# steve-the-bayesian/BOOM

Measured on AMD Instinct MI355X. Metric: Gibbs sweeps/sec (all chains), n=1e4 p=512 spike-slab, higher is better.
Workload: dtype f64; 1 GPU; BregVsSampler spike-and-slab n=1e4 p=512, 1024 chains per GPU, fp64 (BASELINE configs[1]); chains_per_gpu=1024, true_signals=16, burn_in=1000, parallelism=chains sharded, 1 GPU(s), suf_build=single device MFMA syrk

## Files before the change

boom_amd/capi.py:

```python
import ctypes as C
import os

import numpy as np

_HERE = os.path.dirname(os.path.abspath(__file__))
LIB_PATH = os.environ.get("BOOM_AMD_LIB", os.path.join(_HERE, "libboomamd.so"))

_dp = C.POINTER(C.c_double)
_u8p = C.POINTER(C.c_uint8)

SUMMARY_SCALARS = 16


class BoomAmdError(RuntimeError):

    def __init__(self, code, message):
        super().__init__(message)
        self.code = code


class BaConfig(C.Structure):
    _fields_ = [("device", C.c_int32), ("chains", C.c_int32),
                ("chain_offset", C.c_int64), ("seed", C.c_uint64),
                ("max_model_size_hint", C.c_int32), ("reserved", C.c_int32)]
# ... 7 lines not shown
    "ba_engine_destroy": (None, [C.c_void_p]),
    "ba_engine_info": (C.c_int, [C.c_void_p, C.POINTER(C.c_int32),
                                 C.POINTER(C.c_int32), C.POINTER(C.c_int32)]),
    "ba_build_suf_from_xy": (C.c_int, [C.c_void_p, C.c_int64, C.c_int32, _dp, _dp]),
    "ba_build_suf_from_xy_device": (C.c_int, [C.c_void_p, C.c_int64, C.c_int32,
                                              C.c_void_p, C.c_void_p]),
    "ba_suf_block_size": (C.c_size_t, [C.c_int32]),
    "ba_suf_partial_device": (C.c_int, [C.c_void_p, C.c_int64, C.c_int32, C.c_void_p,
                                        C.c_void_p, C.c_void_p]),
    "ba_set_suf_from_block_device": (C.c_int, [C.c_void_p, C.c_int64, C.c_int32, C.c_void_p]),
    "ba_upload_regression_suf": (C.c_int, [C.c_void_p, C.c_int32, _dp, _dp,
                                           C.c_double, C.c_double, C.c_double, _dp]),
    "ba_get_regression_suf": (C.c_int, [C.c_void_p, _dp, _dp, _dp, _dp, _dp, _dp]),
    "ba_set_slab": (C.c_int, [C.c_void_p, _dp, _dp]),
    "ba_set_spike": (C.c_int, [C.c_void_p, _dp, C.c_int64]),
    "ba_set_sigma_prior": (C.c_int, [C.c_void_p, C.c_double, C.c_double, C.c_double]),
    "ba_set_priors_ctor1": (C.c_int, [C.c_void_p, C.c_double, C.c_double,
                                      C.c_double, C.c_int32]),
    "ba_set_priors_ctor2": (C.c_int, [C.c_void_p, C.c_double, C.c_double,
                                      C.c_double, C.c_double, C.c_double, C.c_int32]),
    "ba_get_priors": (C.c_int, [C.c_void_p, _dp, _dp, _dp, _dp, _dp]),
    "ba_set_options": (C.c_int, [C.c_void_p, C.c_int32, C.c_double, C.c_int32, C.c_int32]),
    "ba_set_tuning": (C.c_int, [C.c_void_p, C.c_int32, C.c_int32, C.c_int32]),
    "ba_set_lookahead": (C.c_int, [C.c_void_p, C.c_int32]),
    "ba_draw_next": (C.c_int, [C.c_void_p]),
    "ba_set_state": (C.c_int, [C.c_void_p, C.c_int64, _u8p, _dp, C.c_double]),
    "ba_get_state": (C.c_int, [C.c_void_p, C.c_int64, _u8p, _dp, _dp]),
    "ba_get_states": (C.c_int, [C.c_void_p, _u8p, _dp, _dp]),
    "ba_logpri": (C.c_int, [C.c_void_p, C.c_int64, _dp]),
    "ba_seed": (C.c_int, [C.c_void_p, C.c_uint64]),
    "ba_sweep": (C.c_int, [C.c_void_p, C.c_int32]),
    "ba_sync": (C.c_int, [C.c_void_p]),
    "ba_log_model_prob": (C.c_int, [C.c_void_p, C.c_int32, _u8p, _dp]),
    "ba_set_sigsq": (C.c_int, [C.c_void_p, C.c_int64, C.c_double]),
    "ba_sss_set_slab": (C.c_int, [C.c_void_p, _dp, _dp, C.c_int32, C.c_int32]),
    "ba_sss_sweep": (C.c_int, [C.c_void_p, C.c_int32]),
    "ba_adaptive_set_options": (C.c_int, [C.c_void_p, C.c_int32, C.c_double, C.c_double]),
    "ba_adaptive_sweep": (C.c_int, [C.c_void_p, C.c_int32]),
    "ba_adaptive_get_rates": (C.c_int, [C.c_void_p, C.c_int64, _dp, _dp,
                                        C.POINTER(C.c_uint64)]),
    "ba_reset_summaries": (C.c_int, [C.c_void_p]),
    "ba_get_summaries": (C.c_int, [C.c_void_p, _dp, _dp, _dp, _dp]),
    "ba_summaries_device": (C.c_int, [C.c_void_p, C.c_void_p]),
    "ba_enable_traces": (C.c_int, [C.c_void_p, C.c_int32]),
    "ba_get_traces": (C.c_int, [C.c_void_p, C.c_int32, _dp, _dp, _dp]),
    "ba_enable_draws": (C.c_int, [C.c_void_p, C.c_int32]),
# ... 204 lines not shown
    def set_priors_ctor2(self, prior_sigma_nobs, prior_sigma_guess, prior_beta_nobs,
                         diagonal_shrinkage, prior_inclusion_probability,
                         force_intercept=True):
        self._check(self.lib.ba_set_priors_ctor2(
            self._h, prior_sigma_nobs, prior_sigma_guess, prior_beta_nobs,
            diagonal_shrinkage, prior_inclusion_probability, int(force_intercept)))

    def get_priors(self):
        p = self.p
        b, om, pi = np.zeros(p), np.zeros(p * p), np.zeros(p)
        df, ss = C.c_double(), C.c_double()
        self._check(self.lib.ba_get_priors(self._h, _p(b), _p(om), _p(pi),
                                           C.byref(df), C.byref(ss)))
        return dict(b=b, ominv=om.reshape(p, p).T.copy(), pi=pi, df=df.value, ss=ss.value)

    def set_options(self, max_flips=-1, swap_threshold=0.8, draw_beta=True,
                    draw_sigma=True):
        self._check(self.lib.ba_set_options(self._h, max_flips, swap_threshold,
                                            int(draw_beta), int(draw_sigma)))

    def set_tuning(self, waves_per_chain=0, walk_policy=-1, kcap_start=0):
        self._check(self.lib.ba_set_tuning(self._h, waves_per_chain, walk_policy, kcap_start))

    def set_state(self, gamma, beta=None, sigsq=1.0, chain=-1):
        g = np.ascontiguousarray(gamma, dtype=np.uint8)
        bb = None if beta is None else _f64(beta)
        self._check(self.lib.ba_set_state(self._h, chain, _b(g), _p(bb), sigsq))

    def get_state(self, chain):
        p = self.p
        g = np.zeros(p, np.uint8)
        b = np.zeros(p)
        s = C.c_double()
        self._check(self.lib.ba_get_state(self._h, chain, _b(g), _p(b), C.byref(s)))
        return g, b, s.value

    def get_states(self):
        p, c = self.p, self.chains
        g = np.zeros((c, p), np.uint8)
        b = np.zeros((c, p))
        s = np.zeros(c)
        self._check(self.lib.ba_get_states(self._h, _b(g), _p(b), _p(s)))
        return g, b, s

    def seed(self, seed):
        self._check(self.lib.ba_seed(self._h, seed))
# ... 39 lines not shown
    def adaptive_sweep(self, nsweeps=1, sync=True):
        self._check(self.lib.ba_adaptive_sweep(self._h, nsweeps))
        if sync:
            self.sync()

    def adaptive_get_rates(self, chain):
        b, d = np.zeros(self.p), np.zeros(self.p)
        it = C.c_uint64()
        self._check(self.lib.ba_adaptive_get_rates(self._h, chain, _p(b), _p(d), C.byref(it)))
        return b, d, it.value

    def reset_summaries(self):
        self._check(self.lib.ba_reset_summaries(self._h))

    def get_summaries(self):
        p = self.p
        inc, bs, bs2 = np.zeros(p), np.zeros(p), np.zeros(p)
        sc = np.zeros(SUMMARY_SCALARS)
        self._check(self.lib.ba_get_summaries(self._h, _p(inc), _p(bs), _p(bs2), _p(sc)))
        return dict(inclusion_count=inc, beta_sum=bs, beta_sumsq=bs2,
                    sweeps=sc[0], sigsq_sum=sc[1], sigsq_sumsq=sc[2], k_sum=sc[3],
                    accepts=sc[4], proposals=sc[5], min_margin=sc[6],
                    slot_hits=float(sc[7]), phase_cycles=sc[8:16].copy(),
                    min_multi_margin=float(sc[8]))

    def summaries_device(self, ptr):
        self._check(self.lib.ba_summaries_device(self._h, ptr))

    def enable_traces(self, max_sweeps):
        self._check(self.lib.ba_enable_traces(self._h, max_sweeps))

    def logpri(self, chain=0):
        out = C.c_double()
        self._check(self.lib.ba_logpri(self._h, chain, C.byref(out)))
        return out.value

    def enable_draws(self, max_sweeps):
        self._check(self.lib.ba_enable_draws(self._h, max_sweeps))

    def get_draws(self, chain, nsweeps):
        p = self.p
        g = np.zeros((nsweeps, p), np.uint8)
        b = np.zeros((nsweeps, p))
        s = np.zeros(nsweeps)
        self._check(self.lib.ba_get_draws(self._h, chain, nsweeps, _b(g), _p(b), _p(s)))
        return g, b, s

# ... 489 lines not shown
```

boom_amd/csrc/diag.h:

```cpp
#pragma once

#define BA_STAMP_ADD(ph, last, i, now, T) do { const long long t_ = (long long)(now); (ph)[i] += (T)(t_ - (last)); (last) = t_; } while (0)
#define BA_STAMP_OFF do { } while (0)
#define BA_CORE_CLOCK __builtin_readcyclecounter()

struct StampCtx { long long last; double ph[8]; };

#ifdef BA_STAMPS
#define STAMP_DECL long long st_last = (long long)BA_CORE_CLOCK; double st_ph[8] = {0, 0, 0, 0, 0, 0, 0, 0}
#define STAMP(i) BA_STAMP_ADD(st_ph, st_last, i, BA_CORE_CLOCK, double)
#else
#define STAMP_DECL BA_STAMP_OFF
#define STAMP(i) BA_STAMP_OFF
#endif
#if defined(BA_STAMPS) && defined(BA_STAMPS2)
#define SUBSTAMP(c, i) BA_STAMP_ADD((c).ph, (c).last, i, BA_CORE_CLOCK, double)
#else
#define SUBSTAMP(c, i) BA_STAMP_OFF
#endif
#if defined(BA_STAMPS) && defined(BA_STAMPS3)
#define TSTAMP(c, i) BA_STAMP_ADD((c).ph, (c).last, i, BA_CORE_CLOCK, double)
#else
#define TSTAMP(c, i) BA_STAMP_OFF
#endif
#if defined(BA_STAMPS) && defined(BA_STAMPS4)
#define HSTAMP(c, i) BA_STAMP_ADD((c).ph, (c).last, i, BA_CORE_CLOCK, double)
#else
#define HSTAMP(c, i) BA_STAMP_OFF
#endif
#ifdef BA_PSTAMPS
#define PSTAMP(i) pst[i] = (long long)BA_CORE_CLOCK
#else
#define PSTAMP(i) BA_STAMP_OFF
#endif
#ifdef BA_KSTAMPS
#define KSTAMP(i) BA_STAMP_ADD(kph, klast, i, BA_CORE_CLOCK, long long)
#define SSTAMP(i) BA_STAMP_ADD(kph, klast, i, BA_CORE_CLOCK, long long)
#else
#define KSTAMP(i) BA_STAMP_OFF
#define SSTAMP(i) BA_STAMP_OFF
#endif
#ifdef BA_RSTAMPS
#define RSTAMP(i) BA_STAMP_ADD(rph, rlast, i, wall_clock64(), long long)
#else
#define RSTAMP(i) BA_STAMP_OFF
#endif
```

boom_amd/csrc/engine.hip:

```cpp
#include "engine_internal.h"

namespace boom_amd {

static thread_local std::string g_error = "";

int fail(int code, const std::string &msg) {
  g_error = msg;
  return code;
}

}

namespace {


const char *status_message(int st) {
  switch (st) {
    case CHAIN_NOT_PD:
      return "The posterior information matrix is not positive definite.  "
             "Check your data or consider adjusting your prior.";
    case CHAIN_NEGATIVE_SS:
      return "Illegal data caused negative sum of squares in "
             "Breg::set_reg_post_params.";
    case CHAIN_ILLEGAL_START:
// ... 292 lines not shown
  P.todo = e->dtodo.ptr;
  P.maxk = e->dmaxk.ptr;
  P.trace_idx = e->dtrace_idx.ptr;
  P.model_scratch = e->dmodel.ptr;
  P.table_lp = e->dtab_lp.ptr;
  P.table_kind = e->dtab_kind.ptr;
  P.table_tag = e->dtab_tag.ptr;
  P.table_keep = e->table_ok ? 1 : 0;
  P.model_tag = e->dmodel_tag.ptr;
  P.model_keep = e->model_ok ? 1 : 0;
  P.suf_changed = (e->data_kind == DATA_STATE_SPACE || latent_data(e->data_kind)) ? 1 : 0;
  P.run_limit = 0;
  P.ran = nullptr;
  P.model_scratch_stride = (int64_t)ssvs_scalar_layout(64).total;
  P.big_kcap = e->big_kcap;
  P.big_model = e->dbig_model.ptr;
  P.big_model_stride = e->big_kcap > 0 ? (int64_t)ssvs_scalar_layout(e->big_kcap).total : 0;
  P.big_xs = e->dbig_xs.ptr;
  P.seed_lo = (uint32_t)e->seed;
  P.seed_hi = (uint32_t)(e->seed >> 32);
  P.stream = 0;
  P.mode = e->cur_mode;
  P.walk_policy = e->tune_walk_policy >= 0 ? e->tune_walk_policy : 1;
  if (e->cur_mode == 1) {
    P.slab_scales = e->sss_slab_scales;
    P.stream = 3;
    P.rng_pos = e->dpos_sss.ptr;
    P.draw_sigma = 0;
    P.draw_beta = 1;
    P.cm_start = nullptr;
    P.max_flips = (e->sss_max_flips > 0) ? std::min(e->sss_max_flips, e->p) : e->p;
  }
  if (e->cur_mode == 1 && student_kind(e->data_kind) && !e->student_allow_selection)
    P.max_flips = 0;
  if (e->cur_mode == 1 && column_service(e->data_kind) && e->cols.V.count) {
    P.mode = e->data_kind == DATA_LOGIT ? 2 : 1;
    if (e->data_kind == DATA_MLOGIT) {
      P.mode = 3;
      P.flip_order = e->dml_order.ptr;
      P.wss = e->dml_wss.ptr;
      if (!e->mlogit_select) P.max_flips = 0;
    }
    P.V = e->cols.V.ptr;
    P.v_chain_stride = (int64_t)e->p * e->p;
    P.model_keep = 0;
    P.table_keep = 0;
// ... 872 lines not shown
  e->swap_threshold = swap_threshold;
  e->draw_beta = draw_beta;
  e->draw_sigma = draw_sigma;
  return BA_OK;
}

int ba_set_tuning(ba_engine *e, int32_t waves_per_chain, int32_t walk_policy,
                  int32_t kcap_start) {
  if (!e) return fail(BA_E_INVALID, "null engine");
  if (!(waves_per_chain == 0 || waves_per_chain == 1 || waves_per_chain == 2 || waves_per_chain == 4))
    return fail(BA_E_INVALID, "waves_per_chain must be 0, 1, 2 or 4");
  if (walk_policy < -1 || walk_policy > 3) return fail(BA_E_INVALID, "walk_policy must be in [-1, 3]");
  if (kcap_start < 0) return fail(BA_E_INVALID, "kcap_start must be non-negative");
  MUTATE(e);
  if (e->state_ready) {
    int rc = set_device(e);
    if (!rc) rc = ba_sync(e);
    if (rc) return rc;
  }
  e->tune_waves = waves_per_chain;
  e->tune_walk_policy = walk_policy;
  e->tune_kcap_start = kcap_start;
  e->device_dirty = true;
  return BA_OK;
}

int ba_set_slot_limit(ba_engine *e, int32_t uniforms) {
  if (!e) return fail(BA_E_INVALID, "null engine");
  if (uniforms < 0 || (uniforms & 1)) return fail(BA_E_INVALID, "uniforms must be even and non-negative");
  MUTATE(e);
  e->slot_limit = uniforms;
  return BA_OK;
}

int ba_set_state(ba_engine *e, int64_t chain, const uint8_t *gamma,
                 const double *beta, double sigsq) {
  ENGINE_PROLOGUE(e);
  if (e->p <= 0) return fail(BA_E_STATE, "set the regression data first");
  if (!gamma) return fail(BA_E_INVALID, "null argument");
  const int64_t C = e->cfg.chains;
  if (chain < -1 || chain >= C) return fail(BA_E_INVALID, "chain index out of range");
  if (latent_data(e->data_kind) && !student_kind(e->data_kind) && sigsq != 1.0)
    return fail(BA_E_INVALID, "the binomial samplers' latent data have unit variance: sigsq must be 1");
  if (chain < 0) la_discard(e);
  MUTATE(e);
  if (e->state_ready) {
// ... 873 lines not shown
```

boom_amd/csrc/engine_internal.h:

```cpp
#pragma once
#include <hip/hip_runtime.h>

#include <algorithm>
#include <cmath>
#include <cstdio>
#include <cstdlib>
#include <cstring>
#include <limits>
#include <string>
#include <unordered_map>
#include <vector>

#include "../../include/boom_amd.h"
#include "kalman_params.h"
#include "ktimer.h"
#include "mlogit_params.h"
#include "probit_params.h"
#include "products.h"
#include "quantile_params.h"
#include "ssvs_params.h"
#include "student_params.h"

namespace boom_amd {
hipError_t launch_ssvs_sweep(hipStream_t stream, const SsvsParams &P, int nsweeps);
// ... 169 lines not shown
    int len = 1, avail = 0, served = 0;
    struct Rows { std::vector<double> k, sig, beta; std::vector<uint16_t> idx; };
    std::unordered_map<int64_t, Rows> cache;
    bool synced = false;
    bool pipe = true;
    bool cur_piped = false;
    bool ahead = false;
    int slot = 0;
    hipEvent_t done[2] = {nullptr, nullptr};
    struct Snap {
      DevBuf<uint8_t> gamma;
      DevBuf<double> beta, sigsq, bsum, bsumsq, acc;
      DevBuf<uint16_t> perm;
      DevBuf<uint64_t> pos;
      DevBuf<int32_t> fail;
      DevBuf<uint32_t> inc;
    } snap;
  } la;
  int rec_cap = 64;
  bool big_active = false;
  int big_kcap = 0;
  DevBuf<double> dbig_model, dbig_xs;
  int tune_waves = 0, tune_walk_policy = -1, tune_kcap_start = 0;
  int cur_mode = 0;
  int sss_slab_scales = 1;
  int sss_max_flips = -1;
  double v_scale = 1.0;
  double v_scale_want = 1.0;
  DevBuf<uint64_t> dpos_sss;
  uint64_t seed = 0;
  DevBuf<double> dada_birth, dada_death, dada_ws;
  DevBuf<uint64_t> dada_iter, dpos_ada;
  int ada_max_flips = 100;
  double ada_step = .001, ada_target = .345;

  bool ss_level_set = false, ss_initialized = false;
  int T = 0;
  DevBuf<double> dss_y, dss_X, dss_scratch;
  void *pinned = nullptr;
  size_t pinned_bytes = 0;
  uint64_t api_seq = 1, clean_seq = 0;
  int api_depth = 0;
  DevBuf<double> dss_yt, dss_Xt;
  DevBuf<uint32_t> dss_obs_mask;
  DevBuf<uint8_t> dss_obs;
  DevBuf<double> dxty_c, dyty_c, dnobs_c;
// ... 199 lines not shown
```

boom_amd/csrc/ssvs_device.h:

```cpp
#pragma once
#include <hip/hip_runtime.h>

#include "device_rng.h"
#include "diag.h"
#include "ssvs_params.h"

namespace boom_amd {

namespace {

constexpr int WAVE = 64;
#define BA_INF (__builtin_inf())


#define AS_LDS __attribute__((address_space(3)))
typedef AS_LDS double lds_f64;
typedef AS_LDS uint16_t lds_u16;
typedef AS_LDS uint32_t lds_u32;
typedef AS_LDS uint8_t lds_u8;
template <class T>
__device__ __forceinline__ AS_LDS T *to_lds(unsigned char *generic) {
  return (AS_LDS T *)(uintptr_t)generic;
}
#define AS_CONST __attribute__((address_space(4)))
// ... 96 lines not shown
};

__device__ __forceinline__ void bind_lds(Chain &ch, unsigned char *smem,
                                         const SsvsLds &lay) {
  ch.Lv = to_lds<double>(smem + lay.Lv);
  ch.La = to_lds<double>(smem + lay.La);
  ch.rdv = to_lds<double>(smem + lay.rdv);
  ch.rda = to_lds<double>(smem + lay.rda);
  ch.w = to_lds<double>(smem + lay.w);
  ch.bg = to_lds<double>(smem + lay.bg);
  ch.g = to_lds<uint16_t>(smem + lay.g);
  ch.perm = to_lds<uint16_t>(smem + lay.perm0);
  ch.perm_alt = to_lds<uint16_t>(smem + lay.perm1);
  ch.oth = to_lds<uint16_t>(smem + lay.oth);
  ch.last = to_lds<uint32_t>(smem + lay.last);
  ch.pred = to_lds<uint16_t>(smem + lay.pred);
  ch.gam = to_lds<uint8_t>(smem + lay.gam);
  ch.gam0 = to_lds<uint8_t>(smem + lay.gam0);
  ch.nbr = to_lds<uint8_t>(smem + lay.nbr);
}

__device__ __forceinline__ void chol_blocks2(const Chain &ch, lds_f64 *LA, lds_f64 *rdA,
                                             lds_f64 *LV, lds_f64 *rdV, bool *okA,
                                             bool *okV, double *ldA, double *ldV) {
  const int k = ch.k, i = ch.lane;
  bool oa = true, ov = true;
  for (int j = 0; j < k && (oa || ov); ++j) {
    const bool mine = (i >= j) && (i < k);
    const int ii = mine ? i : j;
    const int jb = j >> 3;
    const int offi = ((ii >> 3) * ((ii >> 3) + 1) / 2) * 64 + (ii & 7) * 8;
    const int offj = (jb * (jb + 1) / 2) * 64 + (j & 7) * 8;
    double sa = LA[bidx(ii, j)], sv = LV[bidx(ii, j)];
    for (int nb = 0; nb < jb; ++nb) {
      typedef double d2_t __attribute__((ext_vector_type(2)));
      const AS_LDS d2_t *pa = (const AS_LDS d2_t *)(LA + offi + nb * 64), *pb = (const AS_LDS d2_t *)(LA + offj + nb * 64);
      const AS_LDS d2_t *pc = (const AS_LDS d2_t *)(LV + offi + nb * 64), *pd = (const AS_LDS d2_t *)(LV + offj + nb * 64);
      d2_t a[4], b[4], c[4], d[4];
#pragma unroll
      for (int t = 0; t < 4; ++t) { a[t] = pa[t]; b[t] = pb[t]; c[t] = pc[t]; d[t] = pd[t]; }
#pragma unroll
      for (int t = 0; t < 4; ++t) {
        sa -= a[t].x * b[t].x;
        sv -= c[t].x * d[t].x;
        sa -= a[t].y * b[t].y;
        sv -= c[t].y * d[t].y;
      }
    }
    {
      const int rem = j & 7;
// ... 26 lines not shown
    }
    if (ov) {
      if (i == j) {
        LV[bidx(j, j)] = sdv;
        rdV[j] = 1.0 / sdv;
      } else if (mine) {
        LV[bidx(i, j)] = sv / sdv;
      }
    }
    wave_sync();
  }
  double la = 0.0, lv = 0.0;
  const double lga = (oa && i < k) ? log(LA[bidx(i, i)]) : 0.0;
  const double lgv = (ov && i < k) ? log(LV[bidx(i, i)]) : 0.0;
  for (int j = 0; j < k; ++j) {
    la += bcast_u(lga, j);
    lv += bcast_u(lgv, j);
  }
  *okA = oa; *okV = ov;
  *ldA = 2.0 * la; *ldV = 2.0 * lv;
}

template <bool REUSE, bool MLVS = false>
__device__ __forceinline__ void refactor(const SsvsParams &P, Chain &ch, Model &M, StampCtx &sx) {
  const int lane = ch.lane, p = ch.p, k = ch.k;
  M.bad = 0;
  M.pd = true;
  double lp;
  const double ldv_in = M.ldv, lda_in = M.lda;
  wave_sync();
  const int kpad = (k + 7) & ~7;
  const int nelem = REUSE ? 0 : kpad * (kpad + 1) / 2;
  const int gm = (lane < k) ? ch.g[lane] : 0;
  const double bm = (lane < k) ? P.b[gm] : 0.0;
  const double xg = (lane < k) ? ch.xty[gm] : 0.0;
  int m0 = 0, n0 = 0;
  double v0 = 0.0, a0 = 0.0;
  if (!REUSE && lane < nelem) {
    int m = (int)((sqrtf(8.0f * (float)lane + 1.0f) - 1.0f) * 0.5f);
    while ((m + 1) * (m + 2) / 2 <= lane) ++m;
    while (m * (m + 1) / 2 > lane) --m;
    m0 = m;
    n0 = lane - m * (m + 1) / 2;
    if (m < k) {
      const size_t o = (size_t)ch.g[m] * p + ch.g[n0];
      v0 = P.V[o] * ch.sv;
      a0 = P.A[o] * ch.sa;
    }
  }
  if (REUSE) {
    lp = M.lp;
  } else {
    double t0 = 0.0, t1 = 0.0;
    if (lane < p) t0 = ch.gam[lane] ? P.l1[lane] : P.l0[lane];
    if (lane + WAVE < p) t1 = ch.gam[lane + WAVE] ? P.l1[lane + WAVE] : P.l0[lane + WAVE];
    double part = 0.0;
    if (lane < p) part += t0;
    if (lane + WAVE < p) part += t1;
    for (int j = lane + 2 * WAVE; j < p; j += WAVE) part += ch.gam[j] ? P.l1[j] : P.l0[j];
    lp = wave_sum(part);
    if (P.max_model_size >= 0 && k > P.max_model_size) lp = -BA_INF;
    if (!(lp > -BA_INF)) lp = -BA_INF;
  }
  M.lp = lp;
  M.ldv = M.lda = M.Q = M.c = 0.0;
  M.SS = ch.ss0q;
  if (k == 0) {
    if constexpr (MLVS) M.logp = lp + ch.k0add;
    else M.logp = ch.mode ? lp : lp - (0.5 * ch.DF - 1.0) * log(ch.ss0q);
    return;
  }
  if (lp == -BA_INF) {
    M.logp = -BA_INF;
    M.pd = false;
    return;
  }
  if (!REUSE && lane < nelem) {
    ch.Lv[bidx(m0, n0)] = v0;
    ch.La[bidx(m0, n0)] = a0;
  }
  for (int e = lane + WAVE; e < nelem; e += WAVE) {
    int m = (int)((sqrtf(8.0f * (float)e + 1.0f) - 1.0f) * 0.5f);
    while ((m + 1) * (m + 2) / 2 <= e) ++m;
    while (m * (m + 1) / 2 > e) --m;
    const int n = e - m * (m + 1) / 2;
    double v = 0.0, a = 0.0;
    if (m < k) {
      const size_t o = (size_t)ch.g[m] * p + ch.g[n];
      v = P.V[o] * ch.sv;
      a = P.A[o] * ch.sa;
    }
    ch.Lv[bidx(m, n)] = v;
    ch.La[bidx(m, n)] = a;
  }
  if (!REUSE && lane < kpad) {
    ch.bg[lane] = bm;
    if (lane >= k) {
      ch.rdv[lane] = 0.0;
      ch.rda[lane] = 0.0;
      ch.w[lane] = 0.0;
    }
  }
  double ab = 0.0;
  unsigned long long nz = __ballot(bm != 0.0);
  while (nz) {
    const int n = __ffsll((long long)nz) - 1;
    nz &= nz - 1;
    const double bn = bcast_u(bm, n);
    const int gn = bcast_u(gm, n);
    if (lane < k) ab += (P.A[(size_t)gm * p + gn] * ch.sa) * bn;
  }
  const double r = (lane < k) ? ab + xg * ch.sx : 0.0;
  M.c = wave_sum(lane < k ? bm * ab : 0.0);
  wave_sync();
  bool okv = true, oka = true;
  if (REUSE) {
    M.lda = lda_in;
    M.ldv = ldv_in;
  } else {
    chol_blocks2(ch, ch.La, ch.rda, ch.Lv, ch.rdv, &oka, &okv, &M.lda, &M.ldv);
  }
  if (!okv) {
    M.pd = false;
    M.logp = -BA_INF;
    return;
  }
  double x = r;
  const double rdm = (lane < k) ? ch.rdv[lane] : 0.0;
#pragma nounroll
  for (int jb = 0; jb * 8 < k; ++jb) {
    double lr[8];
    const int rowm = (lane >= jb * 8 && lane < k) ? lane : jb * 8;
    const int base = bidx(rowm, jb * 8);
#pragma unroll
    for (int t = 0; t < 8; ++t) lr[t] = ch.Lv[base + t];
#pragma unroll
    for (int t = 0; t < 8; ++t) {
      const int j = jb * 8 + t;
      if (j < k) {
        const double wj = bcast_u(x, j) * bcast_u(rdm, j);
        if (lane == j) x = wj;
        else if (lane > j && lane < k) x -= lr[t] * wj;
      }
    }
// ... 4 lines not shown
  wave_sync();
  if (ch.mode) {
    if (!oka) {
      M.lda = -BA_INF;
      M.logp = -BA_INF;
      return;
    }
    M.logp = lp + 0.5 * (M.lda - M.ldv) - 0.5 * (M.c - M.Q);
    return;
  }
  if (!(M.SS >= 0.0) || isinf(M.SS)) {
    M.bad = CHAIN_NEGATIVE_SS;
    M.logp = -BA_INF;
    return;
  }
  if (!oka) {
    M.lda = -BA_INF;
    M.logp = -BA_INF;
    return;
  }
  M.logp = lp + 0.5 * (M.lda - M.ldv) - (0.5 * ch.DF - 1.0) * log(M.SS);
}

__device__ __forceinline__ void apply_flip(Chain &ch, int j) {
  const int lane = ch.lane, k = ch.k;
  const int gm = (lane < k) ? ch.g[lane] : 0x7fffffff;
  const int below = __popcll(__ballot(lane < k && gm < j));
  const bool add = !ch.gam[j];
  wave_sync();
  if (add) {
    const int up = __shfl_up(gm, 1, WAVE);
    if (lane == below) ch.g[lane] = (uint16_t)j;
    else if (lane > below && lane <= k) ch.g[lane] = (uint16_t)up;
    if (lane == 0) ch.gam[j] = 1;
    ch.k = k + 1;
  } else {
    const int dn = __shfl_down(gm, 1, WAVE);
    if (lane >= below && lane < k - 1) ch.g[lane] = (uint16_t)dn;
    if (lane == 0) ch.gam[j] = 0;
    ch.k = k - 1;
  }
  wave_sync();
}

__device__ __forceinline__ void bind_slot(Chain &ch, const SsvsParams &P, int chain, int slot) {
  const size_t c = (size_t)slot * P.chains + chain;
  ch.tab_lp = P.table_lp + c * ch.p;
  ch.tab_kind = P.table_kind + c * ch.p;
  ch.sc_store = P.model_scratch + c * P.model_scratch_stride;
}

template <int NB>
__device__ __forceinline__ void publish_model(Chain &ch, const Model &M) {
  const int lane = ch.lane, k = ch.k;
  constexpr int KCAP = NB * 8;
  const SsvsScalarLayout S = ssvs_scalar_layout(KCAP);
  const int kpad = (k + 7) & ~7;
  const int nblk = (kpad / 8) * (kpad / 8 + 1) / 2;
  double *dst = ch.sc_store;
  for (int e = lane; e < nblk * 64; e += WAVE) {
    dst[S.Lv + e] = ch.Lv[e];
    dst[S.La + e] = ch.La[e];
  }
  if (lane < kpad) {
    dst[S.rdv + lane] = ch.rdv[lane];
// ... 728 lines not shown
```

boom_amd/csrc/ssvs_params.h:

```cpp
#pragma once
#include <stdint.h>

namespace boom_amd {

enum ChainStatus : int32_t {
  CHAIN_OK = 0,
  CHAIN_NOT_PD = 1,
  CHAIN_NEGATIVE_SS = 2,
  CHAIN_ILLEGAL_START = 3,
  CHAIN_RNG_BRANCH = 4,
  CHAIN_FORECAST_VARIANCE = 5,
  CHAIN_MODEL_TOO_LARGE = 6,
  CHAIN_NEED_COLUMN = 7,
  CHAIN_NEED_COLUMN_BIG = 8
};
enum { MLVS_ILLEGAL_START = 12 };

enum { SUMMARY_SCALARS = 16 };
enum {
  ACC_SWEEPS = 0,
  ACC_SIGSQ = 1,
  ACC_SIGSQ2 = 2,
  ACC_K = 3,
  ACC_ACCEPTS = 4,
  ACC_PROPOSALS = 5,
  ACC_MIN_MARGIN = 6,
  ACC_SLOT_HITS = 7,
  ACC_PHASE0 = 8,
  ACC_COUNT = 16
};

struct SsvsParams {
  int32_t p;
  int32_t chains;
  int32_t chain_first;
  int32_t chain_count;
  int64_t chain_offset;
  int32_t kcap;
  int32_t waves;
  int32_t mode;
  int64_t v_chain_stride;
  const uint32_t *col_valid;
  int32_t col_words;
  int32_t *col_request;
  const double *v_diag;
  int32_t walk_policy;
  int32_t slab_scales;

  const double *V;
  const double *A;
  const double *b;
// ... 54 lines not shown
  double ada_step, ada_target;
  int32_t ada_max_flips;
  int32_t *q_in, *q_out;
  int32_t *q_error;
  int32_t trace_row0;
  uint8_t *snap_gamma;
  double *snap_beta, *snap_sigsq, *snap_bsum, *snap_bsumsq, *snap_acc;
  uint16_t *snap_perm;
  uint64_t *snap_pos;
  int32_t *snap_fail;
  uint32_t *snap_inc;
  int32_t adaptive;
  double *ada_ws;

  int32_t big_kcap;
  double *big_model;
  int64_t big_model_stride;
  double *big_xs;
  const double *xty_planes;
  int32_t xty_nplanes;
  int64_t xty_plane_stride;
  const uint16_t *flip_order;
  const double *wss;
};

struct SsvsLds {
  uint32_t Lv, La, rdv, rda, w, bg, ctrl, park, g, perm0, perm1, oth, last, pred, gam, gam0, nbr, total;
};

static inline __host__ __device__ SsvsLds ssvs_lds_layout(int p, int kcap) {
  SsvsLds L;
  const uint32_t nb = (uint32_t)kcap / 8;
  const uint32_t fac = nb * (nb + 1) / 2 * 64 * 8;
  const uint32_t pv = (((uint32_t)p * 2) + 15u) & ~15u;
  uint32_t o = 0;
  L.Lv = o;    o += fac;
  L.La = o;    o += fac;
  L.rdv = o;   o += (uint32_t)kcap * 8;
  L.rda = o;   o += (uint32_t)kcap * 8;
  L.w = o;     o += (uint32_t)kcap * 8;
  L.bg = o;    o += (uint32_t)kcap * 8;
  L.ctrl = o;  o += 512;
  L.park = o;  o += 4 * 512;
  L.g = o;     o += (((uint32_t)kcap * 2) + 15u) & ~15u;
  L.perm0 = o; o += pv;
  L.perm1 = o; o += pv;
// ... 92 lines not shown
```

boom_amd/csrc/ssvs_sweep_body.h:

```cpp
#pragma once
#include "ssvs_device.h"

namespace boom_amd {

template <int NB, int W, int WPE, bool MLVS = false>
__device__ __forceinline__ void ssvs_sweep_body(SsvsParams P, int nsweeps, const int chain,
                                                unsigned char *smem) {
  constexpr bool SHUFFLE_MASKED = NB >= 6 && W > 1;
  P.V += (size_t)chain * (size_t)P.v_chain_stride;
  if (P.col_valid) {
    P.col_valid += (size_t)chain * (size_t)P.col_words;
    P.v_diag += (size_t)chain * (size_t)P.p;
  }
  int tid_ = threadIdx.x;
  BA_OPAQUE_V(tid_);
  int lane = tid_ & (WAVE - 1);
  const int wave = tid_ >> 6;
  const int p = P.p;
#ifdef BA_PSTAMPS
  long long pst[8];
  pst[0] = (long long)__builtin_readcyclecounter();
#endif
  constexpr int FOLD_Z = 16;
  const bool fold = (W == 1) && P.xty_planes != nullptr;
// ... 176 lines not shown
    if (inc && slot < KCAP) ch.g[slot] = (uint16_t)j;
    k += __popcll(mask);
  }
  if (k > KCAP) status = CHAIN_MODEL_TOO_LARGE;
  ch.k = k;
  wave_sync();
  bool aborted = false;
  int need_col = -1;
  int kmax = k;
  int trace_at = (P.trace_row0 >= 0) ? P.trace_row0 : (P.trace_idx ? P.trace_idx[chain] : 0);

  uint64_t pos = uni((uint64_t)P.rng_pos[chain]);
  int failures = uni((int)P.failures[chain]);
  double sigsq = uni((double)P.sigsq[chain]);
  double beta_m = 0.0;
  int gprev = 0, kprev = 0;
  bool beta_valid = false;

  lds_f64 *sum_b = to_lds<double>(smem + lay.park + 512);
  lds_f64 *sum_b2 = to_lds<double>(smem + lay.park + 1024);
  AS_LDS int *sum_n = to_lds<int>(smem + lay.park + 1536);
  AS_LDS int *sum_g = to_lds<int>(smem + lay.park + 1792);
  sum_b[lane] = 0.0; sum_b2[lane] = 0.0; sum_n[lane] = 0; sum_g[lane] = -1;
  if (lane < 8) ctl[CT_ACC + lane] = (lane == ACC_MIN_MARGIN) ? BA_INF : 0.0;
  wave_sync();
#define ACC_ADD(slot, x) do { if (lane == 0) ctl[CT_ACC + (slot)] += (double)(x); } while (0)
#define ACC_MIN(x) do { if (lane == 0) ctl[CT_ACC + ACC_MIN_MARGIN] = fmin(ctl[CT_ACC + ACC_MIN_MARGIN], (x)); } while (0)
  int done = 0;

  const int nflips = P.max_flips;
  STAMP_DECL;
  StampCtx sx;
  sx.last = (long long)__builtin_readcyclecounter();
  for (int i = 0; i < 8; ++i) sx.ph[i] = 0.0;

  Model M;
  M.bad = 0; M.pd = true; M.logp = 0; M.lp = 0; M.ldv = 0; M.lda = 0; M.Q = 0; M.c = 0; M.SS = 0;
  Pending pe;
  pe.kind = EV_INIT; pe.f1 = pe.f2 = -1; pe.lu = 0; pe.lfw = pe.lrev = 0; pe.check_legal = false;
  enum { PH_BEGIN, PH_FLIPS, PH_SWAP, PH_TAIL, PH_JOIN, PH_COMMIT };
  int phase = PH_BEGIN, sweep = 0, i0 = 0;
  bool model_checked = false;
  int perm_sel = 0;
  bool use_table = false;
  int cur = 0, other_var = -1;
  bool other_ok = false, table_valid_other = false;
  const int model_tag_in = P.model_keep ? P.model_tag[chain] : 0;
// ... 20 lines not shown
      const double s0 = sc[0], s1 = sc[1], s2 = sc[2], s3 = sc[3], s4 = sc[4], s5 = sc[5], s6 = sc[6], s7 = sc[7];
      restore_model<NB>(ch);
      M.logp = s0; M.lp = s1; M.ldv = s2; M.lda = s3;
      M.Q = s4; M.c = s5; M.SS = s6; M.pd = s7 != 0.0;
      unsigned long long u = (unsigned long long)ch.sc_store;
      asm volatile("s_dcache_inv\n\ts_waitcnt lgkmcnt(0)" : "+s"(u) : : "memory");
      ch.sc = (c_f64 *)u;
    }
    if (P.suf_changed) {
      refactor<true, MLVS>(P, ch, M, sx);
      if (M.bad) status = M.bad;
      else publish_model<NB>(ch, M);
    }
    if (lane == 0) {
      ctl[CT_LOGP] = M.logp; ctl[CT_LP] = M.lp; ctl[CT_LDV] = M.ldv;
      ctl[CT_LDA] = M.lda; ctl[CT_Q] = M.Q; ctl[CT_C] = M.c;
    }
    wave_sync();
    pe.kind = EV_NONE;
  }

  PSTAMP(4);
  while (status == CHAIN_OK) {
    if constexpr ((W > 1 && !(NB == 4 && W == 2)) || (W == 1 && NB >= 4)) {
      asm volatile("" : "+v"(lane));
      ch.lane = lane;
    }
    if (pe.kind != EV_NONE && !spec) {
      if (pe.kind == EV_FORCE && pe.f2 < 0 && other_ok && pe.f1 == other_var) {
        gam0_fresh = false;
        apply_flip(ch, pe.f1);
        cur ^= 1;
        bind_slot(ch, P, chain, cur);
        restore_model<NB>(ch);
        {
          const SsvsScalarLayout S = ssvs_scalar_layout(KCAP);
          const double *sc = ch.sc_store + S.scal;
          M.logp = sc[0]; M.lp = sc[1]; M.ldv = sc[2]; M.lda = sc[3];
          M.Q = sc[4]; M.c = sc[5]; M.SS = sc[6]; M.pd = sc[7] != 0.0;
          unsigned long long u = (unsigned long long)ch.sc_store;
          asm volatile("s_dcache_inv\n\ts_waitcnt lgkmcnt(0)" : "+s"(u) : : "memory");
          ch.sc = (c_f64 *)u;
        }
        if (lane == 0) {
          ctl[CT_LOGP] = M.logp; ctl[CT_LP] = M.lp; ctl[CT_LDV] = M.ldv;
          ctl[CT_LDA] = M.lda; ctl[CT_Q] = M.Q; ctl[CT_C] = M.c;
        }
        wave_sync();
        {
          const bool t = table_valid;
          table_valid = table_valid_other;
          table_valid_other = t;
        }
        ACC_ADD(ACC_ACCEPTS, 1);
#ifndef BA_STAMPS
        ACC_ADD(ACC_SLOT_HITS, 1);
#endif
        if (!M.pd) status = CHAIN_NOT_PD;
        pe.kind = EV_NONE;
        pe.f1 = pe.f2 = -1;
        pe.lfw = pe.lrev = 0.0;
        pe.check_legal = false;
        STAMP(2);
        continue;
      }
      gam0_fresh = false;
      Model keep;
      keep.logp = M.logp; keep.SS = M.SS; keep.pd = M.pd; keep.bad = M.bad;
      keep.lp = ctl[CT_LP]; keep.ldv = ctl[CT_LDV]; keep.lda = ctl[CT_LDA];
      keep.Q = ctl[CT_Q]; keep.c = ctl[CT_C];
      if (pe.f1 >= 0) apply_flip(ch, pe.f1);
      if (pe.f2 >= 0) apply_flip(ch, pe.f2);
      bool rejected = false;
      {
        Model Mn;
        refactor<false, MLVS>(P, ch, Mn, sx);
        if (Mn.bad) {
          status = Mn.bad;
        } else {
          bool acc = true;
          if (pe.kind == EV_TRY_GE || pe.kind == EV_TRY_LT) {
            const double d = (Mn.logp - pe.lfw) - (keep.logp - pe.lrev);
            if (Mn.logp > -BA_INF) ACC_MIN(fabs(pe.lu - d));
            acc = (pe.kind == EV_TRY_GE) ? !(pe.lu > d) : (pe.lu < d);
          }
          if (acc) {
            M = Mn;
            M.logp = uni(M.logp);
            M.SS = uni(M.SS);
            if (pe.kind != EV_INIT || pe.check_legal) {
              table_valid_other = table_valid;
              table_valid = false;
              other_ok = (pe.kind != EV_INIT) && pe.f1 >= 0 && pe.f2 < 0;
              other_var = pe.f1;
              cur ^= 1;
              bind_slot(ch, P, chain, cur);
            }
            if (pe.kind != EV_INIT) ACC_ADD(ACC_ACCEPTS, 1);
          } else {
// ... 5 lines not shown
            rejected = true;
          }
        }
      }
      if (status == CHAIN_OK) {
        if (!rejected) {
          publish_model<NB>(ch, M);
          if (lane == 0) {
            ctl[CT_LOGP] = M.logp; ctl[CT_LP] = M.lp; ctl[CT_LDV] = M.ldv;
            ctl[CT_LDA] = M.lda; ctl[CT_Q] = M.Q; ctl[CT_C] = M.c;
          }
          wave_sync();
        }
        if (pe.kind == EV_FORCE && !M.pd) status = CHAIN_NOT_PD;
        if (pe.kind == EV_INIT && pe.check_legal &&
            !(M.logp > -BA_INF && M.logp < BA_INF))
          status = CHAIN_ILLEGAL_START;
      }
      pe.kind = EV_NONE;
      pe.f1 = pe.f2 = -1;
      pe.lfw = pe.lrev = 0.0;
      pe.check_legal = false;
      STAMP(2);
      continue;
    }

    if (phase == PH_BEGIN) {
      if (sweep + (commit_pending ? 1 : 0) >= nsweeps) {
        if (!commit_pending) break;
        phase = PH_COMMIT;
        continue;
      }
      {
        const bool ut = (P.walk_policy != 0) && (stops_prev <= 1 || P.walk_policy == 2);
        const bool mc = model_checked || (M.logp > -BA_INF && M.logp < BA_INF);
        const bool will_fork = nflips > 0 && W > 1 && ut && table_valid && mc && p > 1 && P.walk_policy != 3 && P.mode != 2 && !MLVS;
        if (commit_pending && !will_fork) {
          phase = PH_COMMIT;
          continue;
        }
      }
      STAMP(7);
      TSTAMP(sx, 7);
      if (nflips > 0) {
        if (!gam0_fresh || P.mode) {
          for (int j = lane; j < p; j += WAVE) {
// ... 384 lines not shown
          }
        }
      }
      beta_m = y;
      beta_valid = true;
      TSTAMP(sx, 6);
    } else if (P.draw_beta) {
      beta_valid = true;
    }
    STAMP(6);
    after_join = PH_COMMIT;
    phase = spec ? PH_JOIN : PH_COMMIT;
  }

  PSTAMP(5);
  if (W > 1) {
    if (lane == 0) ctl[CT_CMD] = (double)CMD_EXIT;
    __syncthreads();
  }

  wave_sync();
#ifndef BA_STAMPS
  double *acc_row = P.acc + (size_t)chain * ACC_COUNT;
  const double acc_old = (lane < 8) ? acc_row[lane] : 0.0;
#endif
  if (sum_g[lane] >= 0 && sum_n[lane]) {
    const size_t o = (size_t)chain * p + sum_g[lane];
    P.inc_count[o] += (unsigned)sum_n[lane];
    P.beta_sum[o] += sum_b[lane];
    P.beta_sumsq[o] += sum_b2[lane];
  }
  wave_sync();
  {
    const lds_u8 *gsrc = aborted ? ch.gam0 : ch.gam;
    const lds_u16 *psrc = (aborted && p > 1) ? ch.perm_alt : ch.perm;
    for (int j = lane; j < p; j += WAVE) {
      g_gamma[j] = gsrc[j];
      g_perm[j] = psrc[j];
    }
    if (aborted) pos = pos0;
  }
  if (beta_valid) {
    double *g_beta = P.beta + (size_t)chain * p;
    for (int j = lane; j < p; j += WAVE) g_beta[j] = 0.0;
    wave_sync();
    if (lane < kprev) g_beta[gprev] = beta_m;
  } else if (nflips > 0 && done > 0) {
// ... 12 lines not shown
    if (P.ran) P.ran[chain] = done;
    const int tag = KCAP | (cur << 8);
    P.table_tag[chain] = (table_valid && !aborted && status == CHAIN_OK) ? tag : 0;
    P.model_tag[chain] = (!aborted && status == CHAIN_OK) ? tag : 0;
    if (P.trace_idx) P.trace_idx[chain] = trace_at + done;
    if (P.maxk) atomicMax(P.maxk, kmax);
#ifdef BA_STAMPS
    double *a = P.acc + (size_t)chain * ACC_COUNT;
    a[ACC_SWEEPS] += done;
    a[ACC_SIGSQ] += ctl[CT_ACC + ACC_SIGSQ];
    a[ACC_SIGSQ2] += ctl[CT_ACC + ACC_SIGSQ2];
    a[ACC_K] += ctl[CT_ACC + ACC_K];
    a[ACC_ACCEPTS] += ctl[CT_ACC + ACC_ACCEPTS];
    a[ACC_PROPOSALS] += ctl[CT_ACC + ACC_PROPOSALS];
    a[ACC_MIN_MARGIN] = fmin(a[ACC_MIN_MARGIN], ctl[CT_ACC + ACC_MIN_MARGIN]);
#endif
#ifdef BA_PSTAMPS
    PSTAMP(6);
    if (chain == 0 || chain == 517)
      printf("ssvs chain %d: status/todo %lld, plane sum %lld, gamma+scalars %lld, restore+refactor %lld, sweeps %lld, epilogue %lld\n",
             chain, pst[1] - pst[0], pst[2] - pst[1], pst[3] - pst[2], pst[4] - pst[3], pst[5] - pst[4], pst[6] - pst[5]);
#endif
#if defined(BA_STAMPS) && defined(BA_STAMPS4)
#elif defined(BA_STAMPS) && (defined(BA_STAMPS2) || defined(BA_STAMPS3))
    SUBSTAMP(sx, 7);
    for (int i = 0; i < 8; ++i) a[ACC_PHASE0 + i] += sx.ph[i];
#elif defined(BA_STAMPS)
    for (int i = 0; i < 8; ++i) { a[ACC_PHASE0 + i] += st_ph[i]; a[ACC_SLOT_HITS] += st_ph[i]; }
#endif
  }
#ifndef BA_STAMPS
  if (lane < 8) {
    const double inc = (lane == ACC_SWEEPS) ? (double)done : ctl[CT_ACC + lane];
    acc_row[lane] = (lane == ACC_MIN_MARGIN) ? fmin(acc_old, inc) : acc_old + inc;
  }
#endif
}

}
```

include/boom_amd.h:

```cpp
#ifndef BOOM_AMD_H
#define BOOM_AMD_H

#include <stddef.h>
#include <stdint.h>

#ifdef __cplusplus
extern "C" {
#endif

enum {
  BA_OK = 0,
  BA_E_INVALID = -1,
  BA_E_HIP = -2,
  BA_E_NOT_PD = -3,
  BA_E_NEGATIVE_SS = -4,
  BA_E_ILLEGAL_START = -5,
  BA_E_RNG_BRANCH = -6,
  BA_E_FORECAST_VARIANCE = -7,
  BA_E_MODEL_TOO_LARGE = -8,
  BA_E_STATE = -9
};

typedef struct ba_engine ba_engine;

// ... 31 lines not shown

int ba_set_slab(ba_engine *e, const double *prior_mean,
                const double *unscaled_prior_precision);
int ba_set_spike(ba_engine *e, const double *prior_inclusion_probabilities,
                 int64_t max_model_size);
int ba_set_sigma_prior(ba_engine *e, double prior_df, double sigma_guess,
                       double sigma_upper_limit);
int ba_set_priors_ctor1(ba_engine *e, double prior_nobs, double expected_rsq,
                        double expected_model_size,
                        int32_t first_term_is_intercept);
int ba_set_priors_ctor2(ba_engine *e, double prior_sigma_nobs,
                        double prior_sigma_guess, double prior_beta_nobs,
                        double diagonal_shrinkage,
                        double prior_inclusion_probability,
                        int32_t force_intercept);
int ba_get_priors(ba_engine *e, double *prior_mean, double *ominv, double *pi,
                  double *prior_df, double *prior_ss);

int ba_set_options(ba_engine *e, int32_t max_flips, double swap_threshold,
                   int32_t draw_beta, int32_t draw_sigma);

int ba_set_tuning(ba_engine *e, int32_t waves_per_chain, int32_t walk_policy,
                  int32_t kcap_start);
int ba_set_slot_limit(ba_engine *e, int32_t uniforms);

int ba_set_state(ba_engine *e, int64_t chain, const uint8_t *gamma,
                 const double *beta, double sigsq);
int ba_get_state(ba_engine *e, int64_t chain, uint8_t *gamma, double *beta,
                 double *sigsq);
int ba_get_states(ba_engine *e, uint8_t *gamma, double *beta, double *sigsq);
int ba_logpri(ba_engine *e, int64_t chain, double *out);
int ba_seed(ba_engine *e, uint64_t seed);

int ba_sweep(ba_engine *e, int32_t nsweeps);
int ba_sync(ba_engine *e);
int ba_set_lookahead(ba_engine *e, int32_t lookahead);
int ba_draw_next(ba_engine *e);
int ba_log_model_prob(ba_engine *e, int32_t ngamma, const uint8_t *gammas,
                      double *out);

int ba_set_sigsq(ba_engine *e, int64_t chain, double sigsq);
int ba_sss_set_slab(ba_engine *e, const double *mu, const double *precision,
                    int32_t precision_scales_with_sigsq, int32_t max_flips);
int ba_sss_sweep(ba_engine *e, int32_t nsweeps);

int ba_adaptive_set_options(ba_engine *e, int32_t max_flips, double step_size,
// ... 155 lines not shown
```

Baseline: 57.09 million sweeps/s.

## Partially rebuild Cholesky factors after single flips, reusing leading columns

After a single-variable flip, the refactor now keeps the leading q columns of the Cholesky factors, where q is the number of included variables below the flipped index. On a deletion it shifts rows up; on an insertion it solves a triangular system for the new row. It then refactorizes only from column q onward instead of rebuilding the whole factor. This cuts O(k^3) work per proposal, at the cost of extra row-shuffle passes and wave_syncs. The new path is on by default (policy 0) and adds counters for partial rebuilds and kept columns.

```diff
diff --git a/boom_amd/capi.py b/boom_amd/capi.py
--- a/boom_amd/capi.py
+++ b/boom_amd/capi.py
@@ -53,6 +53,7 @@
     "ba_get_priors": (C.c_int, [C.c_void_p, _dp, _dp, _dp, _dp, _dp]),
     "ba_set_options": (C.c_int, [C.c_void_p, C.c_int32, C.c_double, C.c_int32, C.c_int32]),
     "ba_set_tuning": (C.c_int, [C.c_void_p, C.c_int32, C.c_int32, C.c_int32]),
+    "ba_set_rebuild_policy": (C.c_int, [C.c_void_p, C.c_int32]),
     "ba_set_lookahead": (C.c_int, [C.c_void_p, C.c_int32]),
     "ba_draw_next": (C.c_int, [C.c_void_p]),
     "ba_set_state": (C.c_int, [C.c_void_p, C.c_int64, _u8p, _dp, C.c_double]),
@@ -303,6 +304,9 @@
     def set_tuning(self, waves_per_chain=0, walk_policy=-1, kcap_start=0):
         self._check(self.lib.ba_set_tuning(self._h, waves_per_chain, walk_policy, kcap_start))
 
+    def set_rebuild_policy(self, policy):
+        self._check(self.lib.ba_set_rebuild_policy(self._h, int(policy)))
+
     def set_state(self, gamma, beta=None, sigsq=1.0, chain=-1):
         g = np.ascontiguousarray(gamma, dtype=np.uint8)
         bb = None if beta is None else _f64(beta)
@@ -388,7 +392,8 @@
                     sweeps=sc[0], sigsq_sum=sc[1], sigsq_sumsq=sc[2], k_sum=sc[3],
                     accepts=sc[4], proposals=sc[5], min_margin=sc[6],
                     slot_hits=float(sc[7]), phase_cycles=sc[8:16].copy(),
-                    min_multi_margin=float(sc[8]))
+                    min_multi_margin=float(sc[8]),
+                    partial_rebuilds=float(sc[9]), columns_kept=float(sc[10]))
 
     def summaries_device(self, ptr):
         self._check(self.lib.ba_summaries_device(self._h, ptr))
diff --git a/boom_amd/csrc/diag.h b/boom_amd/csrc/diag.h
--- a/boom_amd/csrc/diag.h
+++ b/boom_amd/csrc/diag.h
@@ -28,6 +28,13 @@
 #else
 #define HSTAMP(c, i) BA_STAMP_OFF
 #endif
+#if defined(BA_STAMPS) && defined(BA_STAMPS5)
+#define FSTAMP(c, i) BA_STAMP_ADD((c).ph, (c).last, i, BA_CORE_CLOCK, double)
+#define FCOUNT(c, i, x) do { (c).ph[i] += (double)(x); } while (0)
+#else
+#define FSTAMP(c, i) BA_STAMP_OFF
+#define FCOUNT(c, i, x) BA_STAMP_OFF
+#endif
 #ifdef BA_PSTAMPS
 #define PSTAMP(i) pst[i] = (long long)BA_CORE_CLOCK
 #else
diff --git a/boom_amd/csrc/engine.hip b/boom_amd/csrc/engine.hip
--- a/boom_amd/csrc/engine.hip
+++ b/boom_amd/csrc/engine.hip
@@ -338,6 +338,7 @@
   P.stream = 0;
   P.mode = e->cur_mode;
   P.walk_policy = e->tune_walk_policy >= 0 ? e->tune_walk_policy : 1;
+  P.rebuild_policy = e->tune_rebuild_policy;
   if (e->cur_mode == 1) {
     P.slab_scales = e->sss_slab_scales;
     P.stream = 3;
@@ -1256,6 +1257,13 @@
   e->tune_walk_policy = walk_policy;
   e->tune_kcap_start = kcap_start;
   e->device_dirty = true;
+  return BA_OK;
+}
+
+int ba_set_rebuild_policy(ba_engine *e, int32_t policy) {
+  if (!e) return fail(BA_E_INVALID, "null engine");
+  if (policy != 0 && policy != 1) return fail(BA_E_INVALID, "rebuild_policy must be 0 or 1");
+  e->tune_rebuild_policy = policy;
   return BA_OK;
 }
 
diff --git a/boom_amd/csrc/engine_internal.h b/boom_amd/csrc/engine_internal.h
--- a/boom_amd/csrc/engine_internal.h
+++ b/boom_amd/csrc/engine_internal.h
@@ -215,6 +215,7 @@
   int big_kcap = 0;
   DevBuf<double> dbig_model, dbig_xs;
   int tune_waves = 0, tune_walk_policy = -1, tune_kcap_start = 0;
+  int tune_rebuild_policy = 0;
   int cur_mode = 0;
   int sss_slab_scales = 1;
   int sss_max_flips = -1;
diff --git a/boom_amd/csrc/ssvs_device.h b/boom_amd/csrc/ssvs_device.h
--- a/boom_amd/csrc/ssvs_device.h
+++ b/boom_amd/csrc/ssvs_device.h
@@ -142,10 +142,10 @@
 
 __device__ __forceinline__ void chol_blocks2(const Chain &ch, lds_f64 *LA, lds_f64 *rdA,
                                              lds_f64 *LV, lds_f64 *rdV, bool *okA,
-                                             bool *okV, double *ldA, double *ldV) {
+                                             bool *okV, double *ldA, double *ldV, int j0 = 0) {
   const int k = ch.k, i = ch.lane;
   bool oa = true, ov = true;
-  for (int j = 0; j < k && (oa || ov); ++j) {
+  for (int j = j0; j < k && (oa || ov); ++j) {
     const bool mine = (i >= j) && (i < k);
     const int ii = mine ? i : j;
     const int jb = j >> 3;
@@ -218,15 +218,19 @@
 }
 
 template <bool REUSE, bool MLVS = false>
-__device__ __forceinline__ void refactor(const SsvsParams &P, Chain &ch, Model &M, StampCtx &sx) {
+__device__ __forceinline__ void refactor(const SsvsParams &P, Chain &ch, Model &M, StampCtx &sx,
+                                         int q = -1, bool ins = false) {
   const int lane = ch.lane, p = ch.p, k = ch.k;
+  const bool part = !REUSE && q >= 0;
+  const int q0 = part ? q : 0;
   M.bad = 0;
   M.pd = true;
   double lp;
   const double ldv_in = M.ldv, lda_in = M.lda;
   wave_sync();
   const int kpad = (k + 7) & ~7;
-  const int nelem = REUSE ? 0 : kpad * (kpad + 1) / 2;
+  const int kt = part ? k - q0 : kpad;
+  const int nelem = REUSE ? 0 : kt * (kt + 1) / 2;
   const int gm = (lane < k) ? ch.g[lane] : 0;
   const double bm = (lane < k) ? P.b[gm] : 0.0;
   const double xg = (lane < k) ? ch.xty[gm] : 0.0;
@@ -236,13 +240,19 @@
     int m = (int)((sqrtf(8.0f * (float)lane + 1.0f) - 1.0f) * 0.5f);
     while ((m + 1) * (m + 2) / 2 <= lane) ++m;
     while (m * (m + 1) / 2 > lane) --m;
-    m0 = m;
-    n0 = lane - m * (m + 1) / 2;
-    if (m < k) {
-      const size_t o = (size_t)ch.g[m] * p + ch.g[n0];
+    m0 = m + q0;
+    n0 = lane - m * (m + 1) / 2 + q0;
+    if (m0 < k) {
+      const size_t o = (size_t)ch.g[m0] * p + ch.g[n0];
       v0 = P.V[o] * ch.sv;
       a0 = P.A[o] * ch.sa;
     }
+  }
+  double xv = 0.0, xa = 0.0;
+  if (part && ins && lane < q0) {
+    const size_t o = (size_t)ch.g[q0] * p + gm;
+    xv = P.V[o] * ch.sv;
+    xa = P.A[o] * ch.sa;
   }
   if (REUSE) {
     lp = M.lp;
@@ -271,6 +281,28 @@
     M.pd = false;
     return;
   }
+  if (part) {
+    const bool mv = lane < k && (ins ? lane > q0 : lane >= q0);
+    const int rs = mv ? (ins ? lane - 1 : lane + 1) : q0, rw = mv ? lane : q0;
+    for (int cb = 0; cb * 8 < q0; ++cb) {
+      const int so = bidx(rs, cb * 8), wo = bidx(rw, cb * 8);
+      double tv[8], ta[8];
+#pragma unroll
+      for (int t = 0; t < 8; ++t) { tv[t] = ch.Lv[so + t]; ta[t] = ch.La[so + t]; }
+      wave_sync();
+#pragma unroll
+      for (int t = 0; t < 8; ++t)
+        if (mv && cb * 8 + t < q0) { ch.Lv[wo + t] = tv[t]; ch.La[wo + t] = ta[t]; }
+      wave_sync();
+    }
+    if (lane >= k && lane < kpad) {
+      for (int cb = 0; cb * 8 < kpad; ++cb) {
+        const int wo = bidx(lane, cb * 8);
+#pragma unroll
+        for (int t = 0; t < 8; ++t) { ch.Lv[wo + t] = 0.0; ch.La[wo + t] = 0.0; }
+      }
+    }
+  }
   if (!REUSE && lane < nelem) {
     ch.Lv[bidx(m0, n0)] = v0;
     ch.La[bidx(m0, n0)] = a0;
@@ -279,7 +311,8 @@
     int m = (int)((sqrtf(8.0f * (float)e + 1.0f) - 1.0f) * 0.5f);
     while ((m + 1) * (m + 2) / 2 <= e) ++m;
     while (m * (m + 1) / 2 > e) --m;
-    const int n = e - m * (m + 1) / 2;
+    const int n = e - m * (m + 1) / 2 + q0;
+    m += q0;
     double v = 0.0, a = 0.0;
     if (m < k) {
       const size_t o = (size_t)ch.g[m] * p + ch.g[n];
@@ -308,14 +341,48 @@
   }
   const double r = (lane < k) ? ab + xg * ch.sx : 0.0;
   M.c = wave_sum(lane < k ? bm * ab : 0.0);
+  FSTAMP(sx, 0);
+  if (part && ins) {
+    const double dgv = (lane < q0) ? ch.Lv[bidx(lane, lane)] : 1.0;
+    const double dga = (lane < q0) ? ch.La[bidx(lane, lane)] : 1.0;
+#pragma nounroll
+    for (int jb = 0; jb * 8 < q0; ++jb) {
+      double lv[8], la[8];
+      const int rowm = (lane >= jb * 8 && lane < q0) ? lane : jb * 8;
+      const int base = bidx(rowm, jb * 8);
+#pragma unroll
+      for (int t = 0; t < 8; ++t) { lv[t] = ch.Lv[base + t]; la[t] = ch.La[base + t]; }
+#pragma unroll
+      for (int t = 0; t < 8; ++t) {
+        const int j = jb * 8 + t;
+        if (j < q0) {
+          const double ev = bcast_u(xv, j) / bcast_u(dgv, j);
+          const double ea = bcast_u(xa, j) / bcast_u(dga, j);
+          if (lane == j) {
+            xv = ev;
+            xa = ea;
+          } else if (lane > j && lane < q0) {
+            xv -= lv[t] * ev;
+            xa -= la[t] * ea;
+          }
+        }
+      }
+    }
+    if (lane < q0) {
+      ch.Lv[bidx(q0, lane)] = xv;
+      ch.La[bidx(q0, lane)] = xa;
+    }
+  }
   wave_sync();
+  FSTAMP(sx, 1);
   bool okv = true, oka = true;
   if (REUSE) {
     M.lda = lda_in;
     M.ldv = ldv_in;
   } else {
-    chol_blocks2(ch, ch.La, ch.rda, ch.Lv, ch.rdv, &oka, &okv, &M.lda, &M.ldv);
-  }
+    chol_blocks2(ch, ch.La, ch.rda, ch.Lv, ch.rdv, &oka, &okv, &M.lda, &M.ldv, q0);
+  }
+  FSTAMP(sx, 2);
   if (!okv) {
     M.pd = false;
     M.logp = -BA_INF;
@@ -366,7 +433,7 @@
   M.logp = lp + 0.5 * (M.lda - M.ldv) - (0.5 * ch.DF - 1.0) * log(M.SS);
 }
 
-__device__ __forceinline__ void apply_flip(Chain &ch, int j) {
+__device__ __forceinline__ int apply_flip(Chain &ch, int j) {
   const int lane = ch.lane, k = ch.k;
   const int gm = (lane < k) ? ch.g[lane] : 0x7fffffff;
   const int below = __popcll(__ballot(lane < k && gm < j));
@@ -385,6 +452,7 @@
     ch.k = k - 1;
   }
   wave_sync();
+  return below;
 }
 
 __device__ __forceinline__ void bind_slot(Chain &ch, const SsvsParams &P, int chain, int slot) {
diff --git a/boom_amd/csrc/ssvs_params.h b/boom_amd/csrc/ssvs_params.h
--- a/boom_amd/csrc/ssvs_params.h
+++ b/boom_amd/csrc/ssvs_params.h
@@ -27,6 +27,8 @@
   ACC_MIN_MARGIN = 6,
   ACC_SLOT_HITS = 7,
   ACC_PHASE0 = 8,
+  ACC_PARTIAL_REBUILDS = 9,
+  ACC_COLUMNS_KEPT = 10,
   ACC_COUNT = 16
 };
 
@@ -127,6 +129,7 @@
   int64_t xty_plane_stride;
   const uint16_t *flip_order;
   const double *wss;
+  int32_t rebuild_policy;
 };
 
 struct SsvsLds {
diff --git a/boom_amd/csrc/ssvs_sweep_body.h b/boom_amd/csrc/ssvs_sweep_body.h
--- a/boom_amd/csrc/ssvs_sweep_body.h
+++ b/boom_amd/csrc/ssvs_sweep_body.h
@@ -222,7 +222,7 @@
   AS_LDS int *sum_n = to_lds<int>(smem + lay.park + 1536);
   AS_LDS int *sum_g = to_lds<int>(smem + lay.park + 1792);
   sum_b[lane] = 0.0; sum_b2[lane] = 0.0; sum_n[lane] = 0; sum_g[lane] = -1;
-  if (lane < 8) ctl[CT_ACC + lane] = (lane == ACC_MIN_MARGIN) ? BA_INF : 0.0;
+  if (lane < 11) ctl[CT_ACC + lane] = (lane == ACC_MIN_MARGIN) ? BA_INF : 0.0;
   wave_sync();
 #define ACC_ADD(slot, x) do { if (lane == 0) ctl[CT_ACC + (slot)] += (double)(x); } while (0)
 #define ACC_MIN(x) do { if (lane == 0) ctl[CT_ACC + ACC_MIN_MARGIN] = fmin(ctl[CT_ACC + ACC_MIN_MARGIN], (x)); } while (0)
@@ -289,7 +289,7 @@
 
   PSTAMP(4);
   while (status == CHAIN_OK) {
-    if constexpr ((W > 1 && !(NB == 4 && W == 2)) || (W == 1 && NB >= 4)) {
+    if constexpr ((W > 1 && !(NB == 4 && W == 2)) || (W == 1 && NB >= 4) || (MLVS && NB == 2)) {
       asm volatile("" : "+v"(lane));
       ch.lane = lane;
     }
@@ -336,12 +336,28 @@
       keep.logp = M.logp; keep.SS = M.SS; keep.pd = M.pd; keep.bad = M.bad;
       keep.lp = ctl[CT_LP]; keep.ldv = ctl[CT_LDV]; keep.lda = ctl[CT_LDA];
       keep.Q = ctl[CT_Q]; keep.c = ctl[CT_C];
-      if (pe.f1 >= 0) apply_flip(ch, pe.f1);
+      FSTAMP(sx, 7);
+      const int kold = ch.k;
+      int fq = -1;
+      if (pe.f1 >= 0) fq = apply_flip(ch, pe.f1);
       if (pe.f2 >= 0) apply_flip(ch, pe.f2);
+      const bool fins = ch.k > kold;
+      if (!(P.rebuild_policy == 0 && pe.kind != EV_INIT && pe.f2 < 0 && kold > 0 && ch.k > 0 &&
+            keep.pd && uni(keep.lda) > -BA_INF))
+        fq = -1;
+#ifndef BA_STAMPS
+      if (fq >= 0) {
+        ACC_ADD(ACC_PARTIAL_REBUILDS, 1);
+        ACC_ADD(ACC_COLUMNS_KEPT, fq);
+      }
+#endif
+      FCOUNT(sx, 5, 1);
+      FCOUNT(sx, 6, fq >= 0 ? fq : 0);
       bool rejected = false;
       {
         Model Mn;
-        refactor<false, MLVS>(P, ch, Mn, sx);
+        refactor<false, MLVS>(P, ch, Mn, sx, fq, fins);
+        FSTAMP(sx, 3);
         if (Mn.bad) {
           status = Mn.bad;
         } else {
@@ -393,6 +409,7 @@
       pe.lfw = pe.lrev = 0.0;
       pe.check_legal = false;
       STAMP(2);
+      FSTAMP(sx, 4);
       continue;
     }
 
@@ -823,7 +840,7 @@
   wave_sync();
 #ifndef BA_STAMPS
   double *acc_row = P.acc + (size_t)chain * ACC_COUNT;
-  const double acc_old = (lane < 8) ? acc_row[lane] : 0.0;
+  const double acc_old = (lane < 11) ? acc_row[lane] : 0.0;
 #endif
   if (sum_g[lane] >= 0 && sum_n[lane]) {
     const size_t o = (size_t)chain * p + sum_g[lane];
@@ -882,15 +899,16 @@
              chain, pst[1] - pst[0], pst[2] - pst[1], pst[3] - pst[2], pst[4] - pst[3], pst[5] - pst[4], pst[6] - pst[5]);
 #endif
 #if defined(BA_STAMPS) && defined(BA_STAMPS4)
-#elif defined(BA_STAMPS) && (defined(BA_STAMPS2) || defined(BA_STAMPS3))
+#elif defined(BA_STAMPS) && (defined(BA_STAMPS2) || defined(BA_STAMPS3) || defined(BA_STAMPS5))
     SUBSTAMP(sx, 7);
+    FSTAMP(sx, 7);
     for (int i = 0; i < 8; ++i) a[ACC_PHASE0 + i] += sx.ph[i];
 #elif defined(BA_STAMPS)
     for (int i = 0; i < 8; ++i) { a[ACC_PHASE0 + i] += st_ph[i]; a[ACC_SLOT_HITS] += st_ph[i]; }
 #endif
   }
 #ifndef BA_STAMPS
-  if (lane < 8) {
+  if (lane < 11) {
     const double inc = (lane == ACC_SWEEPS) ? (double)done : ctl[CT_ACC + lane];
     acc_row[lane] = (lane == ACC_MIN_MARGIN) ? fmin(acc_old, inc) : acc_old + inc;
   }
diff --git a/include/boom_amd.h b/include/boom_amd.h
--- a/include/boom_amd.h
+++ b/include/boom_amd.h
@@ -77,6 +77,7 @@
 
 int ba_set_tuning(ba_engine *e, int32_t waves_per_chain, int32_t walk_policy,
                   int32_t kcap_start);
+int ba_set_rebuild_policy(ba_engine *e, int32_t policy);
 int ba_set_slot_limit(ba_engine *e, int32_t uniforms);
 
 int ba_set_state(ba_engine *e, int64_t chain, const uint8_t *gamma,
```

Measured after the change: 60.05 million sweeps/s, median of 6. 5.2% higher.
